# jayleicn/ClipBERT

Hardware: NVIDIA H100
Metric: clips/sec fwd+bwd MSRVTT ret (ResNet50+BERT-base) (higher is better)
Workload: dtype bf16

## Files before the change

### clipbert_b200/csrc/gemm.cu

```cuda
#include <algorithm>

#include "common.cuh"
#include "host_util.h"

namespace cb {

constexpr int BM = 128;
constexpr int BK = 64;
constexpr int CONSUMER_WARPS = 8;
constexpr int GEMM_THREADS = (CONSUMER_WARPS + 1) * 32;
constexpr int PP_THREADS = 3 * 128;
constexpr int PP_PRODUCER_REGS = 40;
constexpr int PP_CONSUMER_REGS = 232;
constexpr int PP_BAR_TURN = 1;
constexpr int MAX_STAGES = 8;
constexpr int SMEM_LIMIT = 232448;
constexpr int STG_PITCH = 36;
constexpr int STG_WARP_FLOATS = 16 * STG_PITCH;
constexpr int EPI_BYTES = CONSUMER_WARPS * STG_WARP_FLOATS * 4;
constexpr int IN_BOX_BYTES = BM * 64 * 2;

struct GemmEpi {
  const float* scale;
  const float* shift;
// ... 215 lines not shown
  const int kc = (K + BK - 1) / BK;
  if (MODE == 1) {
    t.tap = r % ntaps;
    const int split = r / ntaps;
    t.it_begin = split * iters_per_split;
    t.n_iters = min(kc, t.it_begin + iters_per_split) - t.it_begin;
  } else {
    t.tap = 0;
    t.it_begin = 0;
    t.n_iters = ntaps * kc;
  }
  return t;
}

template <int BN, int TA, int TB>
__device__ __forceinline__ void mma_tile(float (&acc)[BN / 2], uint32_t smem0, int stage_bytes, int KCH, int STAGES, int n_iters, int wg,
                                         int lane, int& s, uint32_t& ph, uint64_t* full_bar, uint64_t* empty_bar) {
  using Cfg = GemmCfg<BN>;
  int prev = -1;
  for (int i = 0; i < n_iters; i += KCH) {
    const int nch = min(KCH, n_iters - i);
    mbar_wait(&full_bar[s], ph);
    __syncwarp();
    wgmma_fence();
    wgmma_fence_acc(acc);
    for (int ch = 0; ch < nch; ++ch) {
      const uint32_t a_addr = smem0 + s * stage_bytes + ch * Cfg::STAGE_BYTES + wg * (64 * 128);
      const uint32_t b_addr = smem0 + s * stage_bytes + ch * Cfg::STAGE_BYTES + Cfg::A_BYTES;
#pragma unroll
      for (int k = 0; k < BK / 16; ++k) {
        const uint64_t ad = TA ? gmma_desc(a_addr + k * 2048, BK * 128, 1024) : gmma_desc(a_addr + k * 32, 16, 1024);
        const uint64_t bd = TB ? gmma_desc(b_addr + k * 2048, BK * 128, 1024) : gmma_desc(b_addr + k * 32, 16, 1024);
        wgmma_bf16<BN, TA, TB>(acc, ad, bd, (i > 0 || ch > 0 || k > 0) ? 1u : 0u);
      }
    }
    wgmma_commit();
    wgmma_wait<1>();
    wgmma_fence_acc(acc);
    if (prev >= 0) {
      __syncwarp();
      if (lane == 0) mbar_arrive(&empty_bar[prev]);
    }
    prev = s;
    if (++s == STAGES) { s = 0; ph ^= 1; }
  }
  wgmma_wait<0>();
  wgmma_fence_acc(acc);
  if (prev >= 0) {
    __syncwarp();
    if (lane == 0) mbar_arrive(&empty_bar[prev]);
  }
}

template <int BN, int TB>
__device__ __forceinline__ void mma_tile_pp(float (&acc)[2][BN / 2], uint32_t smem0, int stage_bytes, int KCH, int STAGES, int n_iters,
                                            int lane, int& s, uint32_t& ph, uint64_t* full_bar, uint64_t* empty_bar, int pass_bar,
                                            bool in_stage) {
  using Cfg = GemmCfg<BN>;
  int prev = -1;
  for (int i = 0; i < n_iters; i += KCH) {
    const int nch = min(KCH, n_iters - i);
    mbar_wait_unguarded(&full_bar[s], ph);
    __syncwarp();
    wgmma_fence();
    wgmma_fence_acc(acc[0]);
    wgmma_fence_acc(acc[1]);
    for (int ch = 0; ch < nch; ++ch) {
      const uint32_t a_addr = smem0 + s * stage_bytes + ch * Cfg::STAGE_BYTES;
      const uint32_t b_addr = a_addr + Cfg::A_BYTES;
#pragma unroll
      for (int k = 0; k < BK / 16; ++k) {
        const uint64_t bd = TB ? gmma_desc(b_addr + k * 2048, BK * 128, 1024) : gmma_desc(b_addr + k * 32, 16, 1024);
        const uint32_t accum = (i > 0 || ch > 0 || k > 0) ? 1u : 0u;
#pragma unroll
        for (int h = 0; h < 2; ++h) wgmma_bf16<BN, 0, TB>(acc[h], gmma_desc(a_addr + h * (64 * 128) + k * 32, 16, 1024), bd, accum);
      }
    }
    wgmma_commit();
    wgmma_wait<1>();
    wgmma_fence_acc(acc[0]);
    wgmma_fence_acc(acc[1]);
    if (prev >= 0) {
      __syncwarp();
      mbar_arrive_if(&empty_bar[prev], lane == 0);
    }
    prev = s;
    if (++s == STAGES) { s = 0; ph ^= 1; }
    if (pass_bar && i + KCH >= n_iters) {
      if (in_stage) mbar_wait_unguarded(&full_bar[s], ph);
      named_bar_arrive(pass_bar, 2 * 128);
    }
  }
  wgmma_wait<0>();
  wgmma_fence_acc(acc[0]);
  wgmma_fence_acc(acc[1]);
  if (prev >= 0) {
    __syncwarp();
    mbar_arrive_if(&empty_bar[prev], lane == 0);
  }
}

template <int BN, bool STORE = false>
__device__ __forceinline__ void wgrad_epilogue(const float (&acc)[BN / 2], float* obase, int64_t out_ld, const float* scale, int M, int N, int r0,
                                               int n0, int lane) {
  const int r1 = r0 + 8;
  const float rs0 = (r0 < M && scale) ? scale[r0] : 1.0f;
  const float rs1 = (r1 < M && scale) ? scale[r1] : 1.0f;
#pragma unroll
  for (int j = 0; j < BN / 8; ++j) {
    const int n = n0 + j * 8 + 2 * (lane & 3);
    if (n < N) {
      if constexpr (STORE) {
        if (r0 < M) *reinterpret_cast<float2*>(obase + static_cast<int64_t>(r0) * out_ld + n) = make_float2(acc[4 * j] * rs0, acc[4 * j + 1] * rs0);
        if (r1 < M) *reinterpret_cast<float2*>(obase + static_cast<int64_t>(r1) * out_ld + n) = make_float2(acc[4 * j + 2] * rs1, acc[4 * j + 3] * rs1);
      } else {
        if (r0 < M) red_add_f32x2(obase + static_cast<int64_t>(r0) * out_ld + n, acc[4 * j] * rs0, acc[4 * j + 1] * rs0);
        if (r1 < M) red_add_f32x2(obase + static_cast<int64_t>(r1) * out_ld + n, acc[4 * j + 2] * rs1, acc[4 * j + 3] * rs1);
      }
    }
  }
}

__device__ __forceinline__ uint32_t swz128(uint32_t box, int r, int q) { return box + r * 128 + ((q ^ (r & 7)) << 4); }

template <int BN, int MODE>
__global__ void __launch_bounds__(PP_THREADS, 1)
    gemm_pingpong_kernel(const __grid_constant__ CUtensorMap tmA, const __grid_constant__ CUtensorMap tmB, const __grid_constant__ CUtensorMap tmR,
                         const __grid_constant__ CUtensorMap tmX, int M, int N, int K, int ntaps, int tap_w, int tap_sign, int tiles_m,
                         int tiles_n, int total_tiles, int STAGES, int KCH, int N_IN, GemmEpi epi) {
  static_assert(MODE != 1 && BN <= 128, "TN / NN tiles of 128 x 64 or 128 x 128");
  using Cfg = GemmCfg<BN>;
  extern __shared__ uint8_t smem_raw[];
  uint8_t* smem = reinterpret_cast<uint8_t*>((reinterpret_cast<uintptr_t>(smem_raw) + 1023) & ~static_cast<uintptr_t>(1023));
  const int stage_bytes = KCH * Cfg::STAGE_BYTES;
  const bool has_res = epi.residual != nullptr, has_aux = epi.aux != nullptr;
  constexpr int IN_TILE_BYTES = (BN / 64) * IN_BOX_BYTES;
  const int in_bytes = (has_res + has_aux) * IN_TILE_BYTES;
  uint8_t* in_base = smem + STAGES * stage_bytes;
  uint8_t* stg_base = in_base + N_IN * in_bytes;
  uint64_t* full_bar = reinterpret_cast<uint64_t*>(stg_base + EPI_BYTES);
  uint64_t* empty_bar = full_bar + MAX_STAGES;
  uint64_t* in_full = empty_bar + MAX_STAGES;
  uint64_t* in_empty = in_full + 2;

  const int warp = __shfl_sync(0xffffffffu, static_cast<int>(threadIdx.x >> 5), 0);
  const int lane = threadIdx.x & 31;
  const int unit = blockIdx.x;
  const int n_units = gridDim.x;
  if (threadIdx.x == 0) dbg_stamp(epi, 0);
  pdl_trigger();
  if (threadIdx.x == 0) {
    tma_prefetch_desc(&tmA);
    tma_prefetch_desc(&tmB);
    if (has_res) tma_prefetch_desc(&tmR);
    if (has_aux) tma_prefetch_desc(&tmX);
    for (int s = 0; s < STAGES; ++s) {
      mbar_init(&full_bar[s], 1);
      mbar_init(&empty_bar[s], 4);
    }
    for (int b = 0; b < 2; ++b) {
      mbar_init(&in_full[b], 1);
      mbar_init(&in_empty[b], 4);
    }
    fence_mbar_init();
  }
  __syncthreads();
  const int kc_per_tap = (K + BK - 1) / BK;
  const int n_iters = ntaps * kc_per_tap;
  const bool in_stage = in_bytes && !N_IN;
  const int tile_stages = (n_iters + KCH - 1) / KCH + (in_stage ? 1 : 0);
  pdl_wait();
  if (threadIdx.x == 0) dbg_stamp(epi, 1);

  if (warp < 4) {
    setmaxnreg_dec<PP_PRODUCER_REGS>();
    if (warp == 0 && lane == 0) {
      constexpr int B_BOXES = (MODE == 0) ? 1 : BN / 64;
      int s = 0;
      uint32_t ph = 0;
      auto load_inputs = [&](int tile) {
        const TileInfo t = decode_tile<BN, MODE>(tile, tiles_m, tiles_n, K, ntaps, 0);
        uint64_t* bar;
        uint8_t* dst;
        if (N_IN) {
          const int local = (tile - unit) / n_units;
          const int b = N_IN == 2 ? (local & 1) : 0;
          const int uses = N_IN == 2 ? (local >> 1) : local;
          mbar_wait(&in_empty[b], (static_cast<uint32_t>(uses) & 1u) ^ 1u);
          bar = &in_full[local & 1];
          dst = in_base + b * in_bytes;
        } else {
          mbar_wait(&empty_bar[s], ph ^ 1);
          bar = &full_bar[s];
          dst = smem + s * stage_bytes;
          if (++s == STAGES) { s = 0; ph ^= 1; }
        }
        mbar_expect_tx(bar, in_bytes);
        if (has_res) {
#pragma unroll
          for (int j = 0; j < BN / 64; ++j) tma_load_2d(dst + j * IN_BOX_BYTES, &tmR, bar, t.n0 + j * 64, t.m0);
          dst += IN_TILE_BYTES;
        }
        if (has_aux) {
#pragma unroll
          for (int j = 0; j < BN / 64; ++j) tma_load_2d(dst + j * IN_BOX_BYTES, &tmX, bar, t.n0 + j * 64, t.m0);
        }
      };
      int pend = -1;
      for (int tile = unit; tile < total_tiles; tile += n_units) {
        const TileInfo t = decode_tile<BN, MODE>(tile, tiles_m, tiles_n, K, ntaps, 0);
        const bool inputs_first = tile < unit + N_IN * n_units;
        if (in_bytes && N_IN && inputs_first) load_inputs(tile);
        for (int i = 0; i < n_iters; i += KCH) {
          const int nch = min(KCH, n_iters - i);
          mbar_wait(&empty_bar[s], ph ^ 1);
          mbar_expect_tx(&full_bar[s], nch * Cfg::STAGE_BYTES);
          int tp = 0, kc = i;
          if (ntaps > 1) { tp = i / kc_per_tap; kc = i - tp * kc_per_tap; }
          for (int ch = 0; ch < nch; ++ch) {
            uint8_t* sa = smem + s * stage_bytes + ch * Cfg::STAGE_BYTES;
            uint8_t* sb = sa + Cfg::A_BYTES;
            int shift = 0;
            if (ntaps == 9) shift = tap_sign * ((tp / 3 - 1) * tap_w + (tp % 3 - 1));
            else if (ntaps > 1) shift = tap_sign * tp * tap_w;
            tma_load_2d(sa, &tmA, &full_bar[s], kc * BK, t.m0 + shift);
            if (MODE == 0) {
              tma_load_2d(sb, &tmB, &full_bar[s], tp * K + kc * BK, t.nb0);
            } else if (epi.mn3d) {
              tma_load_3d(sb, &tmB, &full_bar[s], 0, kc * BK, (tp * N + t.nb0) >> 6);
            } else {
#pragma unroll
              for (int j = 0; j < B_BOXES; ++j) tma_load_2d(sb + j * (BK * 128), &tmB, &full_bar[s], tp * N + t.nb0 + j * 64, kc * BK);
            }
            if (++kc == kc_per_tap) { kc = 0; ++tp; }
          }
          if (++s == STAGES) { s = 0; ph ^= 1; }
          if (i == 0 && tile == unit) dbg_stamp(epi, 2);
        }
        if (in_stage) load_inputs(tile);
        if (pend >= 0) load_inputs(pend);
        pend = (in_bytes && N_IN && !inputs_first) ? tile : -1;
      }
      if (pend >= 0) load_inputs(pend);
      dbg_stamp(epi, 3);
    }
    return;
  }

  setmaxnreg_inc<PP_CONSUMER_REGS>();
  const int wg = (warp >> 2) - 1;
  const int wq = warp & 3;
  const uint32_t smem0 = smem_u32(smem);
  const uint64_t dseed = epi.drop_thresh ? drop_seed(epi.seed, epi.seed_off) : 0ull;
  float acc[2][BN / 2];
  int s = 0;
  uint32_t ph = 0;
  auto ring_skip = [&](int n) {
    s += n;
    while (s >= STAGES) { s -= STAGES; ph ^= 1; }
  };
  if (wg == 1) ring_skip(tile_stages);

  const int er = lane & 15, eh = lane >> 4;
  float* stg = reinterpret_cast<float*>(stg_base) + (warp - 4) * STG_WARP_FLOATS;
  const bool has_out2 = epi.out2 != nullptr;
  const bool has_shift = epi.shift != nullptr;
  const bool full = (N & 15) == 0 && epi.scale == nullptr;
  const bool drop = epi.drop_thresh != 0;
  int kind = EK_GENERIC;
  if (full) {
    if (!drop && !has_out2 && !has_aux && (epi.act == CB_ACT_NONE || epi.act == CB_ACT_RELU)) kind = EK_SHIFT_ACT;
    else if (!drop && !has_out2 && !has_shift && has_aux && epi.aux_mode == CB_AUX_RELU_MASK && epi.act == CB_ACT_NONE) kind = EK_RELU_MASK;
    else if (drop && !has_out2 && !has_aux && epi.act == CB_ACT_NONE) kind = EK_DROP_RES;
    else if (!drop && has_out2 && !has_aux && !has_res && epi.act == CB_ACT_GELU_STASH_GRAD) kind = EK_GELU_STASH;
    else if (!drop && !has_out2 && !has_shift && has_aux && epi.aux_mode == CB_AUX_MUL && epi.act == CB_ACT_NONE) kind = EK_AUX_MUL;
  }
  const bool kind_relu = epi.act == CB_ACT_RELU;
  const bool guard = (N & 15) != 0;

  for (int local = wg, tile = unit + wg * n_units; tile < total_tiles; local += 2, tile += 2 * n_units) {
    const TileInfo t = decode_tile<BN, MODE>(tile, tiles_m, tiles_n, K, ntaps, 0);
    if (local > 0) named_bar_sync(PP_BAR_TURN + wg, 2 * 128);
    const int pass = tile + n_units < total_tiles ? PP_BAR_TURN + (wg ^ 1) : 0;
    mma_tile_pp<BN, MODE != 0>(acc, smem0, stage_bytes, KCH, STAGES, n_iters, lane, s, ph, full_bar, empty_bar, pass, in_stage);

    const uint32_t in_buf = N_IN ? smem_u32(in_base) + (N_IN == 2 ? wg : 0) * in_bytes : smem0 + s * stage_bytes;
    if (in_bytes) {
      if (N_IN) mbar_wait_unguarded(&in_full[wg], static_cast<uint32_t>(local >> 1) & 1u);
      else mbar_wait_unguarded(&full_bar[s], ph);
    }
    int orow_half[2];
#pragma unroll
    for (int h = 0; h < 2; ++h) {
      const int m = t.m0 + h * 64 + wq * 16 + er;
      bool row_ok = m < M;
      int64_t orow = m;
      if (epi.rowmap == CB_ROWMAP_PAD) {
        const int hw = epi.H * epi.W;
        const int img = m / hw;
        const int r = m - img * hw;
        const int y = r / epi.W, x = r - y * epi.W;
        orow = (static_cast<int64_t>(img) * (epi.H + 2) + y + 1) * (epi.W + 2) + x + 1;
      } else if (epi.rowmap == CB_ROWMAP_UNPAD) {
        const int wp = epi.W + 2, hp = epi.H + 2;
        const int img = m / (hp * wp);
        const int r = m - img * (hp * wp);
        const int y = r / wp, x = r - y * wp;
        row_ok = row_ok && y >= 1 && y <= epi.H && x >= 1 && x <= epi.W;
        orow = (static_cast<int64_t>(img) * epi.H + (y - 1)) * epi.W + (x - 1);
      }
      orow_half[h] = row_ok ? static_cast<int>(orow) : -1;
    }
#pragma unroll
    for (int sc = 0; sc < BN / 32; ++sc) {
#pragma unroll 1
      for (int h = 0; h < 2; ++h) {
        const int wrow = h * 64 + wq * 16;
        __syncwarp();
#pragma unroll
        for (int jj = 0; jj < 4; ++jj) {
          const int j = sc * 4 + jj;
          float* p = stg + (lane >> 2) * STG_PITCH + jj * 8 + 2 * (lane & 3);
          const bool h1 = h != 0;
          *reinterpret_cast<float2*>(p) = make_float2(h1 ? acc[1][4 * j] : acc[0][4 * j], h1 ? acc[1][4 * j + 1] : acc[0][4 * j + 1]);
          *reinterpret_cast<float2*>(p + 8 * STG_PITCH) =
              make_float2(h1 ? acc[1][4 * j + 2] : acc[0][4 * j + 2], h1 ? acc[1][4 * j + 3] : acc[0][4 * j + 3]);
        }
        __syncwarp();
        const int nb = t.n0 + sc * 32 + eh * 16;
        const int64_t orow = h ? orow_half[1] : orow_half[0];
        if (orow < 0 || nb >= N) continue;
        constexpr int NC = 16;
        float f[NC];
        const uint32_t srow = smem_u32(stg + er * STG_PITCH + eh * 16);
#pragma unroll
        for (int j = 0; j < NC / 4; ++j) {
          const uint4 u = lds128(srow + j * 16);
          f[4 * j] = __uint_as_float(u.x); f[4 * j + 1] = __uint_as_float(u.y);
          f[4 * j + 2] = __uint_as_float(u.z); f[4 * j + 3] = __uint_as_float(u.w);
        }
        uint32_t res16[NC / 2], aux16[NC / 2];
        const int tc = sc * 32 + eh * 16;
        const int q = (tc & 63) >> 3;
        if (has_res) {
#pragma unroll
          for (int j = 0; j < 2; ++j) {
            const uint4 u = lds128(swz128(in_buf + (tc >> 6) * IN_BOX_BYTES, wrow + er, q + j));
            res16[4 * j] = u.x; res16[4 * j + 1] = u.y; res16[4 * j + 2] = u.z; res16[4 * j + 3] = u.w;
          }
        }
        if (has_aux) {
#pragma unroll
          for (int j = 0; j < 2; ++j) {
            const uint4 u = lds128(swz128(in_buf + (has_res ? IN_TILE_BYTES : 0) + (tc >> 6) * IN_BOX_BYTES, wrow + er, q + j));
            aux16[4 * j] = u.x; aux16[4 * j + 1] = u.y; aux16[4 * j + 2] = u.z; aux16[4 * j + 3] = u.w;
          }
        }
        float shv[NC];
        if (has_shift) {
#pragma unroll
          for (int j = 0; j < NC; j += 4) {
            float4 s4 = make_float4(0.f, 0.f, 0.f, 0.f);
            if (nb + j + 4 <= N) s4 = __ldg(reinterpret_cast<const float4*>(epi.shift + nb + j));
            shv[j] = s4.x; shv[j + 1] = s4.y; shv[j + 2] = s4.z; shv[j + 3] = s4.w;
          }
        }
        uint32_t o2_16[NC / 2];
        switch (kind) {
          case EK_SHIFT_ACT: epilogue_shift_act<NC>(f, shv, has_shift, res16, has_res, kind_relu); break;
          case EK_RELU_MASK: epilogue_relu_mask<NC>(f, res16, has_res, aux16); break;
          case EK_DROP_RES:
            epilogue_drop_res<NC>(f, shv, has_shift, res16, has_res, dseed, static_cast<uint64_t>(orow) * static_cast<uint64_t>(N) + nb,
                                  epi.drop_thresh, epi.drop_inv_keep);
            break;
          case EK_GELU_STASH: epilogue_gelu_stash<NC>(f, shv, has_shift, o2_16); break;
          case EK_AUX_MUL: epilogue_aux_mul<NC>(f, res16, has_res, aux16); break;
          default:
            if (guard) epilogue_math<NC, true>(f, epi, shv, has_shift, dseed, nb, N, orow, res16, has_res, aux16, has_aux, o2_16, has_out2);
            else epilogue_math<NC, false>(f, epi, shv, has_shift, dseed, nb, N, orow, res16, has_res, aux16, has_aux, o2_16, has_out2);
        }
        if (epi.out_fp32) {
          float* o = reinterpret_cast<float*>(epi.out) + orow * epi.out_ld + nb;
#pragma unroll
          for (int j = 0; j < NC; j += 4)
            if (nb + j + 4 <= N) *reinterpret_cast<float4*>(o + j) = make_float4(f[j], f[j + 1], f[j + 2], f[j + 3]);
        } else {
          __nv_bfloat16* o = reinterpret_cast<__nv_bfloat16*>(epi.out) + orow * epi.out_ld + nb;
#pragma unroll
          for (int j = 0; j < 2; ++j)
            if (nb + 8 * j + 8 <= N)
              *reinterpret_cast<uint4*>(o + 8 * j) = make_uint4(pack_bf16x2(f[8 * j], f[8 * j + 1]), pack_bf16x2(f[8 * j + 2], f[8 * j + 3]),
                                                                pack_bf16x2(f[8 * j + 4], f[8 * j + 5]), pack_bf16x2(f[8 * j + 6], f[8 * j + 7]));
        }
        if (has_out2) {
          __nv_bfloat16* o = epi.out2 + orow * epi.out2_ld + nb;
#pragma unroll
          for (int j = 0; j < 2; ++j)
            if (nb + 8 * j + 8 <= N) *reinterpret_cast<uint4*>(o + 8 * j) = make_uint4(o2_16[4 * j], o2_16[4 * j + 1], o2_16[4 * j + 2], o2_16[4 * j + 3]);
        }
      }
    }
    if (in_bytes) {
      __syncwarp();
      if (lane == 0) mbar_arrive(N_IN ? &in_empty[N_IN == 2 ? wg : 0] : &empty_bar[s]);
      if (!N_IN && ++s == STAGES) { s = 0; ph ^= 1; }
    }
    ring_skip(tile_stages);
  }
  if (threadIdx.x == 4 * 32) dbg_stamp(epi, 11);
}

template <int BN, bool DET = false>
__global__ void __launch_bounds__(GEMM_THREADS, 1)
    gemm_kernel(const __grid_constant__ CUtensorMap tmA, const __grid_constant__ CUtensorMap tmB, int M, int N, int K, int ntaps, int tap_w,
                int tap_sign, int iters_per_split, int tiles_m, int tiles_n, int total_tiles, int STAGES, int KCH, GemmEpi epi, float* ws) {
  using Cfg = GemmCfg<BN>;
  extern __shared__ uint8_t smem_raw[];
  uint8_t* smem = reinterpret_cast<uint8_t*>((reinterpret_cast<uintptr_t>(smem_raw) + 1023) & ~static_cast<uintptr_t>(1023));
  const int stage_bytes = KCH * Cfg::STAGE_BYTES;
  uint64_t* full_bar = reinterpret_cast<uint64_t*>(smem + STAGES * stage_bytes);
  uint64_t* empty_bar = full_bar + MAX_STAGES;

  const int warp = __shfl_sync(0xffffffffu, static_cast<int>(threadIdx.x >> 5), 0);
  const int lane = threadIdx.x & 31;
  const int unit = blockIdx.x;
  const int n_units = gridDim.x;
  if (threadIdx.x == 0) dbg_stamp(epi, 0);
  pdl_trigger();
  if (threadIdx.x == 0) {
    tma_prefetch_desc(&tmA);
    tma_prefetch_desc(&tmB);
    for (int s = 0; s < STAGES; ++s) {
      mbar_init(&full_bar[s], 1);
      mbar_init(&empty_bar[s], CONSUMER_WARPS);
    }
    fence_mbar_init();
  }
  __syncthreads();
  pdl_wait();
  if (threadIdx.x == 0) dbg_stamp(epi, 1);

  if (warp >= CONSUMER_WARPS) {
    if (warp == CONSUMER_WARPS && lane == 0) {
      int s = 0;
      uint32_t ph = 0;
      for (int tile = unit; tile < total_tiles; tile += n_units) {
        const TileInfo t = decode_tile<BN, 1>(tile, tiles_m, tiles_n, K, ntaps, iters_per_split);
        int shift = 0;
        if (ntaps == 9) shift = tap_sign * ((t.tap / 3 - 1) * tap_w + (t.tap % 3 - 1));
        for (int i = 0; i < t.n_iters; i += KCH) {
          const int nch = min(KCH, t.n_iters - i);
          mbar_wait(&empty_bar[s], ph ^ 1);
          mbar_expect_tx(&full_bar[s], nch * Cfg::STAGE_BYTES);
          int kit = t.it_begin + i;
          for (int ch = 0; ch < nch; ++ch, ++kit) {
            uint8_t* sa = smem + s * stage_bytes + ch * Cfg::STAGE_BYTES;
            uint8_t* sb = sa + Cfg::A_BYTES;
            const int p = kit * BK;
            if (epi.mn3d) {
              tma_load_3d(sa, &tmA, &full_bar[s], 0, p, t.m0 >> 6);
              tma_load_3d(sb, &tmB, &full_bar[s], 0, p + shift, t.nb0 >> 6);
            } else {
// ... 86 lines not shown
  const SmemPlan none = plan_ring(bn, staging, kiters, force_kch, 0, 0);
  if (in_bytes == 0) return none;
  const SmemPlan two = plan_ring(bn, staging, kiters, force_kch, in_bytes, 2);
  if (two.stages >= 2 && two.stages * two.kch >= kiters) return two;
  if (kiters > 4 && none.stages >= 2 && none.kch * none.chunk_bytes >= in_bytes) return none;
  return plan_ring(bn, staging, kiters, force_kch, in_bytes, 1);
}
static int epi_in_bytes(const cb_gemm_desc& d, int bn) {
  return d.mode == CB_GEMM_WGRAD ? 0 : ((d.residual != nullptr) + (d.aux != nullptr)) * (bn / 64) * IN_BOX_BYTES;
}

static int real_splits(int kc, int want) {
  const int sp = want < 1 ? 1 : (want > kc ? kc : want);
  return ceil_div(kc, ceil_div(kc, sp));
}

struct SplitReduceJob {
  float* out;
  const float* ws;
  int64_t out_ld;
  int M, W, S;
};
struct SplitReduce {
  int njobs;
  SplitReduceJob j[8];
};
__global__ void __launch_bounds__(256) wgrad_split_reduce_kernel(const __grid_constant__ SplitReduce r) {
  pdl_wait();
  pdl_trigger();
  const SplitReduceJob& J = r.j[blockIdx.y];
  const int w4 = J.W / 4;
  const int64_t total = static_cast<int64_t>(J.M) * w4, plane = static_cast<int64_t>(J.M) * J.W;
  for (int64_t i = static_cast<int64_t>(blockIdx.x) * 256 + threadIdx.x; i < total; i += static_cast<int64_t>(gridDim.x) * 256) {
    const int64_t m = i / w4;
    const int c = static_cast<int>(i - m * w4) * 4;
    float4* o = reinterpret_cast<float4*>(J.out + m * J.out_ld + c);
    float4 v = *o;
    const float* p = J.ws + m * J.W + c;
    for (int s = 0; s < J.S; ++s) {
      const float4 a = *reinterpret_cast<const float4*>(p + s * plane);
      v.x += a.x; v.y += a.y; v.z += a.z; v.w += a.w;
    }
    *o = v;
  }
}
static int launch_split_reduce(const SplitReduce& r, cudaStream_t stream, const char* what) {
  int64_t most = 0;
  for (int i = 0; i < r.njobs; ++i) most = std::max(most, static_cast<int64_t>(r.j[i].M) * (r.j[i].W / 4));
  const int gx = static_cast<int>(std::min<int64_t>(1024, (most + 255) / 256));
  launch_k(wgrad_split_reduce_kernel, dim3(gx, r.njobs), 256, 0, stream, r);
  return check_launch(what);
}

template <int BN, int MODE, bool DET = false>
static int launch_gemm(const cb_gemm_desc& d, const GemmEpi& epi_in, cudaStream_t stream, float* ws = nullptr) {
  static_assert(MODE == 1 || BN <= 128, "TN / NN: 128 x 64 or 128 x 128 tiles");
  static_assert(MODE == 1 || !DET, "only the weight gradients have a deterministic instantiation");
  GemmEpi epi = epi_in;
  using Cfg = GemmCfg<BN>;
  static bool attr_set = false;
  auto kern = [] {
    if constexpr (MODE == 1) return gemm_kernel<BN, DET>;
    else return gemm_pingpong_kernel<BN, MODE>;
  }();
  if (!attr_set) {
    cudaError_t e = cudaFuncSetAttribute(kern, cudaFuncAttributeMaxDynamicSharedMemorySize, SMEM_LIMIT);
    if (e != cudaSuccess) {
      set_error("cudaFuncSetAttribute(smem=%d): %s", SMEM_LIMIT, cudaGetErrorString(e));
      return CB_ERR_CUDA;
    }
    attr_set = true;
  }
  alignas(64) CUtensorMap ta, tb, tr, tx;
  bool mn3d = false;
  int iters_per_split = 0;
  const int tiles_m = ceil_div(d.m, BM), tiles_n = ceil_div(d.n, BN);
  int total = tiles_m * tiles_n;
  int kiters;
  bool ok;
  if (MODE == 0) {
    ok = get_tmap_2d(&ta, d.a, d.k, d.a_rows, d.a_ld, BK, BM) &&
         get_tmap_2d(&tb, d.b, static_cast<uint64_t>(d.k) * d.ntaps, d.b_rows, d.b_ld, BK, BN);
    kiters = ceil_div(d.k, BK) * d.ntaps;
  } else if (MODE == 2) {
    ok = get_tmap_2d(&ta, d.a, d.k, d.a_rows, d.a_ld, BK, BM);
    mn3d = g_mn3d && d.n % 64 == 0 &&
           get_tmap_3d_mn(&tb, d.b, static_cast<uint64_t>(d.n) * d.ntaps, d.b_rows, d.b_ld, BK, BN / 64);
    if (!mn3d) ok = ok && get_tmap_2d(&tb, d.b, static_cast<uint64_t>(d.n) * d.ntaps, d.b_rows, d.b_ld, 64, BK);
    kiters = ceil_div(d.k, BK) * d.ntaps;
  } else {
    mn3d = g_mn3d && d.m % 64 == 0 && d.n % 64 == 0 && get_tmap_3d_mn(&ta, d.a, d.m, d.a_rows, d.a_ld, BK, BM / 64) &&
           get_tmap_3d_mn(&tb, d.b, d.n, d.b_rows, d.b_ld, BK, BN / 64);
    ok = mn3d || (get_tmap_2d(&ta, d.a, d.m, d.a_rows, d.a_ld, 64, BK) && get_tmap_2d(&tb, d.b, d.n, d.b_rows, d.b_ld, 64, BK));
    const int kc = ceil_div(d.k, BK);
    iters_per_split = ceil_div(kc, real_splits(kc, d.split_k));
    total *= real_splits(kc, d.split_k) * d.ntaps;
    kiters = iters_per_split;
  }
  tr = ta;
  tx = ta;
  if (MODE != 1 && d.residual) ok = ok && get_tmap_2d(&tr, d.residual, d.n, d.m, d.res_ld, 64, BM);
  if (MODE != 1 && d.aux) ok = ok && get_tmap_2d(&tx, d.aux, d.n, d.m, d.aux_ld, 64, BM);
  if (!ok) return CB_ERR_CUDA;
  epi.mn3d = mn3d ? 1 : 0;
  const int units = sm_count();
  const int grid = total < units ? total : units;
  const int in_bytes = epi_in_bytes(d, BN);
  const SmemPlan sp = plan_smem(BN, MODE != 1, kiters, (d.reserved >> 8) & 15, in_bytes);
  const int kch = sp.kch, stages = sp.stages;
  if (stages < 2) {
    set_error("cb_gemm: not enough shared memory for a 2-stage pipeline (BN=%d, epilogue %d B + inputs %d B)", BN, sp.epi_bytes,
              in_bytes);
    return CB_ERR_INVALID;
  }
  const int smem_bytes = stages * kch * Cfg::STAGE_BYTES + sp.n_in * in_bytes + sp.epi_bytes + Cfg::BAR_BYTES + 1024;
  if constexpr (MODE == 1)
    launch_gemm_k(kern, grid, GEMM_THREADS, smem_bytes, stream, ta, tb, d.m, d.n, d.k, d.ntaps, d.tap_w, d.tap_sign, iters_per_split,
                  tiles_m, tiles_n, total, stages, kch, epi, ws);
  else
    launch_gemm_k(kern, grid, PP_THREADS, smem_bytes, stream, ta, tb, tr, tx, d.m, d.n, d.k, d.ntaps, d.tap_w, d.tap_sign, tiles_m,
                  tiles_n, total, stages, kch, sp.n_in, epi);
  return check_launch("cb_gemm");
}

struct LaunchCfg {
  int bn, splits;
};

static LaunchCfg choose_config(const cb_gemm_desc& d, int units) {
  const int kc = ceil_div(d.k, BK);
  const bool wgrad = d.mode == CB_GEMM_WGRAD;
  const int block_n = (!wgrad && d.block_n == 256) ? 128 : d.block_n;
  static const int cand[3] = {64, 128, 256};
  LaunchCfg best = {64, 1};
  double best_cost = 1e30;
  for (int c = 0; c < 3; ++c) {
    const int bn = cand[c];
    if (block_n && bn != block_n) continue;
    if (!wgrad && bn == 256) continue;
    if (bn > 64 && d.n <= bn / 2) continue;
    const int64_t base = static_cast<int64_t>(ceil_div(d.m, BM)) * ceil_div(d.n, bn) * (wgrad ? d.ntaps : 1);
    const int max_split = wgrad ? (d.split_k > 0 ? d.split_k : (kc < 32 ? kc : 32)) : 1;
    for (int sp = (wgrad && d.split_k > 0) ? d.split_k : 1; sp <= max_split; ++sp) {
      const int ips = ceil_div(wgrad ? kc : kc * d.ntaps, sp);
      const int real_sp = wgrad ? ceil_div(kc, ips) : 1;
      const int64_t tiles = base * real_sp;
      const double rounds = static_cast<double>((tiles + units - 1) / units);
      const SmemPlan pl = plan_smem(bn, !wgrad, ips, (d.reserved >> 8) & 15, epi_in_bytes(d, bn));
      if (pl.stages < 2) continue;
      const double shallow = (pl.stages * pl.kch < 3 && ips > 2) ? 3.0 : 1.0;
      const double stage_cost = 450.0 + pl.kch * pl.chunk_bytes / 60.0;
      const double main_loop = ceil_div(ips, pl.kch) * stage_cost * shallow;
      double cost;
      if (wgrad) {
        cost = rounds * (main_loop + bn * 24.0) + 2500.0;
      } else {
        const double epi = bn * 30.0;
        const double per_tile = main_loop > 0.5 * (main_loop + epi) ? main_loop : 0.5 * (main_loop + epi);
        cost = rounds * per_tile + 0.5 * epi + 2500.0;
      }
      if (cost < best_cost) {
        best_cost = cost;
        best = {bn, real_sp};
      }
    }
  }
  return best;
}

constexpr int WG_MAX_PROBLEMS = 8;
struct WgradProblem {
  CUtensorMap tmA, tmB;
  float* out;
  const float* scale;
  int64_t out_ld;
  int M, N, K;
  int ntaps, tap_w, tap_sign;
  int iters_per_split, tiles_m, tiles_n;
  int tile_begin;
  int mn3d;
};
struct WgradGroup {
  int nprob, total_tiles;
  WgradProblem p[WG_MAX_PROBLEMS];
};
struct WgradWorkspace {
  float* p[WG_MAX_PROBLEMS];
};
struct WgTile {
  int pi, m0, n0, tap, it_begin, n_iters;
};
__device__ __forceinline__ WgTile wg_decode(const WgradGroup& g, int tile) {
  WgTile t;
  int pi = 0;
  while (pi + 1 < g.nprob && tile >= g.p[pi + 1].tile_begin) ++pi;
  const WgradProblem& P = g.p[pi];
  int r = tile - P.tile_begin;
  const int nt = r % P.tiles_n;
  r /= P.tiles_n;
  const int mt = r % P.tiles_m;
  r /= P.tiles_m;
  t.pi = pi;
  t.m0 = mt * BM;
  t.tap = r % P.ntaps;
  const int split = r / P.ntaps;
  const int kc = (P.K + BK - 1) / BK;
  t.it_begin = split * P.iters_per_split;
  t.n_iters = min(kc, t.it_begin + P.iters_per_split) - t.it_begin;
  t.n0 = nt;
  return t;
}

template <int BN, bool DET = false>
__global__ void __launch_bounds__(GEMM_THREADS, 1)
    wgrad_group_kernel(const __grid_constant__ WgradGroup g, int STAGES, int KCH, const __grid_constant__ WgradWorkspace ws) {
  using Cfg = GemmCfg<BN>;
  extern __shared__ uint8_t smem_raw[];
  uint8_t* smem = reinterpret_cast<uint8_t*>((reinterpret_cast<uintptr_t>(smem_raw) + 1023) & ~static_cast<uintptr_t>(1023));
// ... 189 lines not shown
extern "C" int cb_gemm(const cb_gemm_desc* dp, void* stream_v) {
  using namespace cb;
  CB_REQUIRE(dp != nullptr, "cb_gemm: null descriptor");
  const cb_gemm_desc& d = *dp;
  cudaStream_t stream = static_cast<cudaStream_t>(stream_v);
  CB_REQUIRE(d.a && d.b && d.out, "cb_gemm: null operand pointer");
  CB_REQUIRE(d.m > 0 && d.n > 0 && d.k > 0, "cb_gemm: empty problem m=%d n=%d k=%d", d.m, d.n, d.k);
  CB_REQUIRE(d.ntaps == 1 || d.ntaps == 9 || (d.ntaps == 4 && d.mode == CB_GEMM_TN),
             "cb_gemm: ntaps must be 1, 9 (3x3 conv) or 4 (row taps, TN only) (got %d)", d.ntaps);
  CB_REQUIRE(d.mode == CB_GEMM_TN || d.mode == CB_GEMM_WGRAD || d.mode == CB_GEMM_NN, "cb_gemm: bad mode %d", d.mode);
  CB_REQUIRE(d.dropout_p >= 0.0f && d.dropout_p <= 1.0f, "cb_gemm: dropout_p %g outside [0, 1]", d.dropout_p);

  GemmEpi epi;
  epi.scale = d.scale;
  epi.shift = d.shift;
  epi.residual = static_cast<const __nv_bfloat16*>(d.residual);
  epi.aux = static_cast<const __nv_bfloat16*>(d.aux);
  epi.aux_mode = d.aux ? d.aux_mode : CB_AUX_NONE;
  epi.act = d.act;
  epi.out = d.out;
  epi.out_ld = d.out_ld;
  epi.out_fp32 = d.out_fp32;
  epi.out2 = static_cast<__nv_bfloat16*>(d.out2);
  epi.out2_ld = d.out2_ld;
  epi.rowmap = d.rowmap;
  epi.H = d.map_h;
  epi.W = d.map_w;
  epi.seed = d.dropout_seed;
  epi.dbg = g_gemm_timeline;
  epi.mn3d = 0;
  {
    const DropCfg dc = make_drop(d.dropout_p, d.dropout_seed);
    epi.drop_thresh = dc.thresh;
    epi.drop_inv_keep = dc.inv_keep;
    epi.seed_off = dc.offset;
  }

  if (d.mode == CB_GEMM_TN || d.mode == CB_GEMM_NN) {
    const bool nn = d.mode == CB_GEMM_NN;
    CB_REQUIRE(d.n % 8 == 0, "cb_gemm(TN): n must be a multiple of 8 (got %d)", d.n);
    CB_REQUIRE(d.k % 8 == 0, "cb_gemm(TN): k must be a multiple of 8 (got %d)", d.k);
    CB_REQUIRE(d.out_ld % 8 == 0, "cb_gemm(TN): out_ld must be a multiple of 8");
    CB_REQUIRE(!d.residual || d.res_ld % 8 == 0, "cb_gemm(TN): res_ld must be a multiple of 8");
    CB_REQUIRE(!d.aux || d.aux_ld % 8 == 0, "cb_gemm(TN): aux_ld must be a multiple of 8");
    CB_REQUIRE((reinterpret_cast<uintptr_t>(d.residual) & 15) == 0, "cb_gemm(TN): residual must be 16-byte aligned");
    CB_REQUIRE((reinterpret_cast<uintptr_t>(d.aux) & 15) == 0, "cb_gemm(TN): aux must be 16-byte aligned");
    CB_REQUIRE(!d.out2 || d.out2_ld % 8 == 0, "cb_gemm(TN): out2_ld must be a multiple of 8");
    CB_REQUIRE(!(d.out2 && d.out_fp32), "cb_gemm(TN): out2 requires a bf16 primary output");
    CB_REQUIRE(d.rowmap == CB_ROWMAP_NONE || (d.map_h > 0 && d.map_w > 0), "cb_gemm: rowmap needs map_h/map_w");
    CB_REQUIRE(d.ntaps == 1 || d.tap_w > 2, "cb_gemm: tap modes need tap_w (padded row pitch in pixels)");
    CB_REQUIRE(d.block_n == 0 || d.block_n == 64 || d.block_n == 128 || d.block_n == 256, "cb_gemm: block_n must be 0, 64, 128 or 256 (got %d)",
               d.block_n);
    const LaunchCfg lc = choose_config(d, sm_count());
    switch (lc.bn) {
      case 64: return nn ? launch_gemm<64, 2>(d, epi, stream) : launch_gemm<64, 0>(d, epi, stream);
      case 128: return nn ? launch_gemm<128, 2>(d, epi, stream) : launch_gemm<128, 0>(d, epi, stream);
      default: CB_REQUIRE(false, "cb_gemm: no tile width for block_n %d", d.block_n);
    }
  } else {
    CB_REQUIRE(d.out_fp32 == 1, "cb_gemm(WGRAD): output must be fp32");
    CB_REQUIRE(d.m % 8 == 0 && d.n % 8 == 0, "cb_gemm(WGRAD): m, n must be multiples of 8 (got %d, %d)", d.m, d.n);
    CB_REQUIRE(d.out_ld % 4 == 0, "cb_gemm(WGRAD): out_ld must be a multiple of 4");
    CB_REQUIRE((reinterpret_cast<uintptr_t>(d.out) & 15) == 0, "cb_gemm(WGRAD): out must be 16-byte aligned");
    const LaunchCfg lc = choose_config(d, plan_sm_count());
    cb_gemm_desc d2 = d;
    d2.split_k = lc.splits;
    if (g_det.load(std::memory_order_relaxed) && lc.splits > 1) {
      const int64_t need = wgrad_ws_bytes(d, lc.splits);
      CB_REQUIRE(d.workspace != nullptr && d.workspace_bytes >= need && (reinterpret_cast<uintptr_t>(d.workspace) & 15) == 0,
                 "cb_gemm(WGRAD): deterministic mode needs a 16-byte aligned workspace of %lld bytes (cb_gemm_workspace_bytes), got %lld",
                 static_cast<long long>(need), static_cast<long long>(d.workspace ? d.workspace_bytes : 0));
      float* ws = static_cast<float*>(d.workspace);
      int rc = CB_ERR_INVALID;
      switch (lc.bn) {
        case 64: rc = launch_gemm<64, 1, true>(d2, epi, stream, ws); break;
        case 128: rc = launch_gemm<128, 1, true>(d2, epi, stream, ws); break;
        case 256: rc = launch_gemm<256, 1, true>(d2, epi, stream, ws); break;
        default: CB_REQUIRE(false, "cb_gemm(WGRAD): block_n must be 0, 64, 128 or 256 (got %d)", lc.bn);
      }
      if (rc != CB_OK) return rc;
      SplitReduce red;
      red.njobs = 1;
      red.j[0] = {static_cast<float*>(d.out), ws, d.out_ld, d.m, d.ntaps * d.n, lc.splits};
      return launch_split_reduce(red, stream, "cb_gemm(split reduce)");
    }
    switch (lc.bn) {
      case 64: return launch_gemm<64, 1>(d2, epi, stream);
      case 128: return launch_gemm<128, 1>(d2, epi, stream);
      case 256: return launch_gemm<256, 1>(d2, epi, stream);
      default: CB_REQUIRE(false, "cb_gemm(WGRAD): block_n must be 0, 64, 128 or 256 (got %d)", lc.bn);
    }
  }
  return CB_ERR_INVALID;
}

extern "C" int cb_gemm_wgrad_group(const cb_gemm_desc* descs, int n, void* stream_v) {
  using namespace cb;
  CB_REQUIRE(descs != nullptr && n >= 1, "cb_gemm_wgrad_group: no problems");
  cudaStream_t stream = static_cast<cudaStream_t>(stream_v);
  for (int i = 0; i < n; ++i) {
    const cb_gemm_desc& d = descs[i];
    CB_REQUIRE(d.mode == CB_GEMM_WGRAD && d.out_fp32 == 1, "cb_gemm_wgrad_group: problem %d is not an fp32 WGRAD descriptor", i);
    CB_REQUIRE(d.a && d.b && d.out && d.m > 0 && d.n > 0 && d.k > 0, "cb_gemm_wgrad_group: problem %d: null operand / empty shape", i);
    CB_REQUIRE(d.m % 8 == 0 && d.n % 8 == 0 && d.out_ld % 4 == 0 && (reinterpret_cast<uintptr_t>(d.out) & 15) == 0,
               "cb_gemm_wgrad_group: problem %d: m, n multiples of 8, out 16-byte aligned, out_ld a multiple of 4", i);
    CB_REQUIRE(d.ntaps == 1 || d.ntaps == 9, "cb_gemm_wgrad_group: problem %d: ntaps must be 1 or 9", i);
  }
  const bool det = g_det.load(std::memory_order_relaxed);
  int64_t need = 0;
  if (det) {
    need = group_ws_bytes(descs, n);
// ... 43 lines not shown
```

### clipbert_b200/ops.py

```python
import ctypes

import torch

from . import _lib as L
from ._lib import (ACT_GELU, ACT_GELU_STASH_GRAD, ACT_NONE, ACT_RELU, ACT_TANH, AUX_GELU_GRAD, AUX_MUL, AUX_NONE,
                   AUX_RELU_MASK, AUX_TANH_GRAD, CB_GEMM_TN, CB_GEMM_WGRAD, ROWMAP_NONE, ROWMAP_PAD, ROWMAP_UNPAD)

CB_GEMM_NN = 2
_c = ctypes
_vp, _i, _i64, _f, _u64 = _c.c_void_p, _c.c_int, _c.c_int64, _c.c_float, _c.c_uint64

_SIGS = {
    "cb_layernorm_fwd": [_vp, _vp, _vp, _vp, _vp, _i, _i, _f, _vp],
    "cb_layernorm_bwd": [_vp, _vp, _vp, _vp, _vp, _vp, _vp, _vp, _vp, _i, _i, _f, _u64, _vp],
    "cb_embed_text_fwd": [_vp, _vp, _vp, _vp, _vp, _vp, _vp, _vp, _i, _i, _i, _i, _i, _f, _f, _u64, _vp],
    "cb_embed_text_bwd": [_vp] * 12 + [_i, _i, _i, _i, _i, _f, _u64, _vp],
    "cb_embed_visual_fwd": [_vp, _vp, _i, _vp, _vp, _vp, _vp, _vp, _vp, _vp, _i, _i, _i, _i, _i, _i, _i, _f, _f, _u64, _vp],
    "cb_embed_visual_bwd": [_vp, _vp, _vp, _vp, _i] + [_vp] * 12 + [_i, _i, _i, _i, _i, _i, _i, _i, _f, _u64, _vp],
    "cb_colsum": [_vp, _i64, _vp, _i, _i, _vp],
    "cb_dropout": [_vp, _vp, _i64, _f, _u64, _vp],
    "cb_dropout_offset_advance": [_vp, _vp, _vp],
    "cb_gelu_bwd": [_vp, _vp, _vp, _i64, _vp],
    "cb_pad_cast": [_vp, _i64, _vp, _i, _i, _i, _vp],
    "cb_cast_scale": [_vp, _vp, _i64, _vp, _i64, _vp],
# ... 226 lines not shown
            if k in _GEMM_PTR_FIELDS:
                v = _p(v) if isinstance(v, torch.Tensor) else v
            setattr(d, k, v)
    return arr


def gemm_workspace_bytes(kw):
    return int(L.lib().cb_gemm_workspace_bytes(_gemm_descs([kw])))


def gemm_wgrad_group_workspace_bytes(kws):
    return int(L.lib().cb_gemm_wgrad_group_workspace_bytes(_gemm_descs(kws), len(kws)))


def _with_workspace(kw, nbytes):
    if nbytes <= 0:
        return kw
    ws, nb = _scratch_args(nbytes, kw["out"])
    return dict(kw, workspace=ws, workspace_bytes=nb)


def _launch_gemm(name, kws):
    arr = _gemm_descs(kws)
    timing = _gemm_timing is not None or _op_timing is not None
    if timing:
        e0, e1 = torch.cuda.Event(enable_timing=True), torch.cuda.Event(enable_timing=True)
        e0.record()
    if name == "cb_gemm":
        rc = L.lib().cb_gemm(arr, _s())
    else:
        rc = L.lib().cb_gemm_wgrad_group(arr, len(kws), _s())
    if rc != 0:
        raise RuntimeError("%s failed (%d): %s" % (name, rc, L.lib().cb_last_error().decode()))
    if timing:
        e1.record()
        if _gemm_timing is not None:
            _gemm_timing.append((e0, e1))
        if _op_timing is not None:
            d = arr[0]
            label = ("gemm mode=%d m=%d n=%d k=%d taps=%d res=%d aux=%d o2=%d f32=%d rm=%d" % (
                d.mode, d.m, d.n, d.k, d.ntaps, bool(d.residual), bool(d.aux), bool(d.out2), d.out_fp32, d.rowmap)
                if name == "cb_gemm" else "gemm wgrad group x%d" % len(kws))
            _op_timing.append((label, e0, e1))


def gemm(**kw):
    if _tuning is None:
        _load_tuning()
    if _gemm_record is not None:
        _gemm_record.append(dict(kw))
    if _tuning and "block_n" not in kw and "reserved" not in kw:
        t = _tuning.get(gemm_key(kw))
        if t is not None:
            kw = dict(kw, block_n=t[0], split_k=t[1], reserved=(t[2] << 8) | (32 if (len(t) > 3 and t[3]) else 0))
    if kw.get("mode", CB_GEMM_TN) == CB_GEMM_WGRAD and deterministic():
        kw = _with_workspace(kw, gemm_workspace_bytes(kw))
    _launch_gemm("cb_gemm", [kw])


group_wgrad = 3


def gemm_wgrad_group(kws):
    if not kws:
        return
    if len(kws) == 1:
        for kw in kws:
            gemm(**kw)
        return
    if _gemm_record is not None:
        _gemm_record.append(dict(group=[dict(kw) for kw in kws]))
    kws = list(kws)
    if deterministic():
        kws[0] = _with_workspace(kws[0], gemm_wgrad_group_workspace_bytes(kws))
    _launch_gemm("cb_gemm_wgrad_group", kws)


def wgrad_split(m, n, k, ntaps=1, block_n=128):
    return 0


def layernorm_fwd(x, gamma, beta, y, stats, eps):
    _call("cb_layernorm_fwd", _p(x), _p(gamma), _p(beta), _p(y), _p(stats), x.shape[0], x.shape[1], eps, _s())


def layernorm_bwd(dy, x, stats, gamma, dx, dx_drop, dgamma, dbeta, dbias_drop, p, seed):
    if (dgamma is not None or dbeta is not None or dbias_drop is not None) and deterministic():
        layernorm_bwd_det(dy, x, stats, gamma, dx, dx_drop, dgamma, dbeta, dbias_drop, p, seed,
                          _scratch(layernorm_bwd_scratch_bytes(x.shape[0]), x))
        return
    _call("cb_layernorm_bwd", _p(dy), _p(x), _p(stats), _p(gamma), _p(dx), _p(dx_drop), _p(dgamma), _p(dbeta),
          _p(dbias_drop), x.shape[0], x.shape[1], p, seed, _s())


def layernorm_bwd_scratch_bytes(m):
    return int(_fn("cb_layernorm_bwd_scratch_bytes")(m))


def layernorm_bwd_det(dy, x, stats, gamma, dx, dx_drop, dgamma, dbeta, dbias_drop, p, seed, scratch):
    _call("cb_layernorm_bwd_det", _p(dy), _p(x), _p(stats), _p(gamma), _p(dx), _p(dx_drop), _p(dgamma), _p(dbeta),
          _p(dbias_drop), x.shape[0], x.shape[1], p, seed, _p(scratch), scratch.numel() * 4, _s())


def embed_text_fwd(ids, word, pos, type0, gamma, beta, out, stats, nseq, lt, l, eps, p, seed):
    _call("cb_embed_text_fwd", _p(ids), _p(word), _p(pos), _p(type0), _p(gamma), _p(beta), _p(out), _p(stats), nseq, lt, l,
          word.shape[0], word.shape[1], eps, p, seed, _s())

# ... 194 lines not shown
```

Baseline: 3987.

## Add cooperative two-warpgroup GEMM kernel for TN/NN with 128x256 tiles

```diff
diff --git a/clipbert_b200/csrc/gemm.cu b/clipbert_b200/csrc/gemm.cu
--- a/clipbert_b200/csrc/gemm.cu
+++ b/clipbert_b200/csrc/gemm.cu
@@ -291,10 +291,10 @@
   }
 }
 
-template <int BN, int TB>
-__device__ __forceinline__ void mma_tile_pp(float (&acc)[2][BN / 2], uint32_t smem0, int stage_bytes, int KCH, int STAGES, int n_iters,
-                                            int lane, int& s, uint32_t& ph, uint64_t* full_bar, uint64_t* empty_bar, int pass_bar,
-                                            bool in_stage) {
+template <int BN, int TB, int NH>
+__device__ __forceinline__ void mma_tile_pp(float (&acc)[NH][BN / 2], uint32_t a_off, uint32_t smem0, int stage_bytes, int KCH, int STAGES,
+                                            int n_iters, int lane, int& s, uint32_t& ph, uint64_t* full_bar, uint64_t* empty_bar,
+                                            int pass_bar, bool in_stage) {
   using Cfg = GemmCfg<BN>;
   int prev = -1;
   for (int i = 0; i < n_iters; i += KCH) {
@@ -302,23 +302,23 @@
     mbar_wait_unguarded(&full_bar[s], ph);
     __syncwarp();
     wgmma_fence();
-    wgmma_fence_acc(acc[0]);
-    wgmma_fence_acc(acc[1]);
+#pragma unroll
+    for (int h = 0; h < NH; ++h) wgmma_fence_acc(acc[h]);
     for (int ch = 0; ch < nch; ++ch) {
-      const uint32_t a_addr = smem0 + s * stage_bytes + ch * Cfg::STAGE_BYTES;
-      const uint32_t b_addr = a_addr + Cfg::A_BYTES;
+      const uint32_t a_addr = smem0 + s * stage_bytes + ch * Cfg::STAGE_BYTES + a_off;
+      const uint32_t b_addr = smem0 + s * stage_bytes + ch * Cfg::STAGE_BYTES + Cfg::A_BYTES;
 #pragma unroll
       for (int k = 0; k < BK / 16; ++k) {
         const uint64_t bd = TB ? gmma_desc(b_addr + k * 2048, BK * 128, 1024) : gmma_desc(b_addr + k * 32, 16, 1024);
         const uint32_t accum = (i > 0 || ch > 0 || k > 0) ? 1u : 0u;
 #pragma unroll
-        for (int h = 0; h < 2; ++h) wgmma_bf16<BN, 0, TB>(acc[h], gmma_desc(a_addr + h * (64 * 128) + k * 32, 16, 1024), bd, accum);
+        for (int h = 0; h < NH; ++h) wgmma_bf16<BN, 0, TB>(acc[h], gmma_desc(a_addr + h * (64 * 128) + k * 32, 16, 1024), bd, accum);
       }
     }
     wgmma_commit();
     wgmma_wait<1>();
-    wgmma_fence_acc(acc[0]);
-    wgmma_fence_acc(acc[1]);
+#pragma unroll
+    for (int h = 0; h < NH; ++h) wgmma_fence_acc(acc[h]);
     if (prev >= 0) {
       __syncwarp();
       mbar_arrive_if(&empty_bar[prev], lane == 0);
@@ -331,8 +331,8 @@
     }
   }
   wgmma_wait<0>();
-  wgmma_fence_acc(acc[0]);
-  wgmma_fence_acc(acc[1]);
+#pragma unroll
+  for (int h = 0; h < NH; ++h) wgmma_fence_acc(acc[h]);
   if (prev >= 0) {
     __syncwarp();
     mbar_arrive_if(&empty_bar[prev], lane == 0);
@@ -362,12 +362,13 @@
 
 __device__ __forceinline__ uint32_t swz128(uint32_t box, int r, int q) { return box + r * 128 + ((q ^ (r & 7)) << 4); }
 
-template <int BN, int MODE>
-__global__ void __launch_bounds__(PP_THREADS, 1)
-    gemm_pingpong_kernel(const __grid_constant__ CUtensorMap tmA, const __grid_constant__ CUtensorMap tmB, const __grid_constant__ CUtensorMap tmR,
-                         const __grid_constant__ CUtensorMap tmX, int M, int N, int K, int ntaps, int tap_w, int tap_sign, int tiles_m,
-                         int tiles_n, int total_tiles, int STAGES, int KCH, int N_IN, GemmEpi epi) {
-  static_assert(MODE != 1 && BN <= 128, "TN / NN tiles of 128 x 64 or 128 x 128");
+template <int BN, int MODE, bool COOP>
+__device__ __forceinline__ void gemm_tn_nn_body(const CUtensorMap& tmA, const CUtensorMap& tmB, const CUtensorMap& tmR, const CUtensorMap& tmX,
+                                                int M, int N, int K, int ntaps, int tap_w, int tap_sign, int tiles_m, int tiles_n,
+                                                int total_tiles, int STAGES, int KCH, int N_IN, const GemmEpi& epi) {
+  static_assert(MODE != 1 && (COOP ? (BN == 128 || BN == 256) : BN <= 128), "TN / NN: ping-pong 128 x 64 / 128, cooperative 128 x 128 / 256");
+  constexpr int READERS = COOP ? 8 : 4;
+  constexpr int NH = COOP ? 1 : 2;
   using Cfg = GemmCfg<BN>;
   extern __shared__ uint8_t smem_raw[];
   uint8_t* smem = reinterpret_cast<uint8_t*>((reinterpret_cast<uintptr_t>(smem_raw) + 1023) & ~static_cast<uintptr_t>(1023));
@@ -395,11 +396,11 @@
     if (has_aux) tma_prefetch_desc(&tmX);
     for (int s = 0; s < STAGES; ++s) {
       mbar_init(&full_bar[s], 1);
-      mbar_init(&empty_bar[s], 4);
+      mbar_init(&empty_bar[s], READERS);
     }
     for (int b = 0; b < 2; ++b) {
       mbar_init(&in_full[b], 1);
-      mbar_init(&in_empty[b], 4);
+      mbar_init(&in_empty[b], READERS);
     }
     fence_mbar_init();
   }
@@ -491,14 +492,14 @@
   const int wq = warp & 3;
   const uint32_t smem0 = smem_u32(smem);
   const uint64_t dseed = epi.drop_thresh ? drop_seed(epi.seed, epi.seed_off) : 0ull;
-  float acc[2][BN / 2];
+  float acc[NH][BN / 2];
   int s = 0;
   uint32_t ph = 0;
   auto ring_skip = [&](int n) {
     s += n;
     while (s >= STAGES) { s -= STAGES; ph ^= 1; }
   };
-  if (wg == 1) ring_skip(tile_stages);
+  if (!COOP && wg == 1) ring_skip(tile_stages);
 
   const int er = lane & 15, eh = lane >> 4;
   float* stg = reinterpret_cast<float*>(stg_base) + (warp - 4) * STG_WARP_FLOATS;
@@ -517,15 +518,18 @@
   const bool kind_relu = epi.act == CB_ACT_RELU;
   const bool guard = (N & 15) != 0;
 
-  for (int local = wg, tile = unit + wg * n_units; tile < total_tiles; local += 2, tile += 2 * n_units) {
+  constexpr int TILE_STEP = COOP ? 1 : 2;
+  for (int local = COOP ? 0 : wg, tile = unit + local * n_units; tile < total_tiles; local += TILE_STEP, tile += TILE_STEP * n_units) {
     const TileInfo t = decode_tile<BN, MODE>(tile, tiles_m, tiles_n, K, ntaps, 0);
-    if (local > 0) named_bar_sync(PP_BAR_TURN + wg, 2 * 128);
-    const int pass = tile + n_units < total_tiles ? PP_BAR_TURN + (wg ^ 1) : 0;
-    mma_tile_pp<BN, MODE != 0>(acc, smem0, stage_bytes, KCH, STAGES, n_iters, lane, s, ph, full_bar, empty_bar, pass, in_stage);
-
-    const uint32_t in_buf = N_IN ? smem_u32(in_base) + (N_IN == 2 ? wg : 0) * in_bytes : smem0 + s * stage_bytes;
+    if (!COOP && local > 0) named_bar_sync(PP_BAR_TURN + wg, 2 * 128);
+    const int pass = (!COOP && tile + n_units < total_tiles) ? PP_BAR_TURN + (wg ^ 1) : 0;
+    mma_tile_pp<BN, MODE != 0, NH>(acc, COOP ? wg * (64 * 128) : 0, smem0, stage_bytes, KCH, STAGES, n_iters, lane, s, ph, full_bar,
+                                   empty_bar, pass, in_stage);
+
+    const int ib = COOP ? (local & 1) : wg;
+    const uint32_t in_buf = N_IN ? smem_u32(in_base) + (N_IN == 2 ? ib : 0) * in_bytes : smem0 + s * stage_bytes;
     if (in_bytes) {
-      if (N_IN) mbar_wait_unguarded(&in_full[wg], static_cast<uint32_t>(local >> 1) & 1u);
+      if (N_IN) mbar_wait_unguarded(&in_full[ib], static_cast<uint32_t>(local >> 1) & 1u);
       else mbar_wait_unguarded(&full_bar[s], ph);
     }
     int orow_half[2];
@@ -553,17 +557,18 @@
 #pragma unroll
     for (int sc = 0; sc < BN / 32; ++sc) {
 #pragma unroll 1
-      for (int h = 0; h < 2; ++h) {
+      for (int h = COOP ? wg : 0; h < (COOP ? wg + 1 : 2); ++h) {
         const int wrow = h * 64 + wq * 16;
         __syncwarp();
 #pragma unroll
         for (int jj = 0; jj < 4; ++jj) {
           const int j = sc * 4 + jj;
           float* p = stg + (lane >> 2) * STG_PITCH + jj * 8 + 2 * (lane & 3);
-          const bool h1 = h != 0;
-          *reinterpret_cast<float2*>(p) = make_float2(h1 ? acc[1][4 * j] : acc[0][4 * j], h1 ? acc[1][4 * j + 1] : acc[0][4 * j + 1]);
+          const bool h1 = !COOP && h != 0;
+          *reinterpret_cast<float2*>(p) =
+              make_float2(h1 ? acc[NH - 1][4 * j] : acc[0][4 * j], h1 ? acc[NH - 1][4 * j + 1] : acc[0][4 * j + 1]);
           *reinterpret_cast<float2*>(p + 8 * STG_PITCH) =
-              make_float2(h1 ? acc[1][4 * j + 2] : acc[0][4 * j + 2], h1 ? acc[1][4 * j + 3] : acc[0][4 * j + 3]);
+              make_float2(h1 ? acc[NH - 1][4 * j + 2] : acc[0][4 * j + 2], h1 ? acc[NH - 1][4 * j + 3] : acc[0][4 * j + 3]);
         }
         __syncwarp();
         const int nb = t.n0 + sc * 32 + eh * 16;
@@ -641,12 +646,27 @@
     }
     if (in_bytes) {
       __syncwarp();
-      if (lane == 0) mbar_arrive(N_IN ? &in_empty[N_IN == 2 ? wg : 0] : &empty_bar[s]);
+      if (lane == 0) mbar_arrive(N_IN ? &in_empty[N_IN == 2 ? ib : 0] : &empty_bar[s]);
       if (!N_IN && ++s == STAGES) { s = 0; ph ^= 1; }
     }
-    ring_skip(tile_stages);
+    if (!COOP) ring_skip(tile_stages);
   }
   if (threadIdx.x == 4 * 32) dbg_stamp(epi, 11);
+}
+
+template <int BN, int MODE>
+__global__ void __launch_bounds__(PP_THREADS, 1)
+    gemm_pingpong_kernel(const __grid_constant__ CUtensorMap tmA, const __grid_constant__ CUtensorMap tmB, const __grid_constant__ CUtensorMap tmR,
+                         const __grid_constant__ CUtensorMap tmX, int M, int N, int K, int ntaps, int tap_w, int tap_sign, int tiles_m,
+                         int tiles_n, int total_tiles, int STAGES, int KCH, int N_IN, GemmEpi epi) {
+  gemm_tn_nn_body<BN, MODE, false>(tmA, tmB, tmR, tmX, M, N, K, ntaps, tap_w, tap_sign, tiles_m, tiles_n, total_tiles, STAGES, KCH, N_IN, epi);
+}
+template <int BN, int MODE>
+__global__ void __launch_bounds__(PP_THREADS, 1)
+    gemm_coop_kernel(const __grid_constant__ CUtensorMap tmA, const __grid_constant__ CUtensorMap tmB, const __grid_constant__ CUtensorMap tmR,
+                     const __grid_constant__ CUtensorMap tmX, int M, int N, int K, int ntaps, int tap_w, int tap_sign, int tiles_m,
+                     int tiles_n, int total_tiles, int STAGES, int KCH, int N_IN, GemmEpi epi) {
+  gemm_tn_nn_body<BN, MODE, true>(tmA, tmB, tmR, tmX, M, N, K, ntaps, tap_w, tap_sign, tiles_m, tiles_n, total_tiles, STAGES, KCH, N_IN, epi);
 }
 
 template <int BN, bool DET = false>
@@ -839,15 +859,17 @@
   return check_launch(what);
 }
 
-template <int BN, int MODE, bool DET = false>
+template <int BN, int MODE, bool DET = false, bool COOP = false>
 static int launch_gemm(const cb_gemm_desc& d, const GemmEpi& epi_in, cudaStream_t stream, float* ws = nullptr) {
-  static_assert(MODE == 1 || BN <= 128, "TN / NN: 128 x 64 or 128 x 128 tiles");
+  static_assert(MODE == 1 || (COOP ? BN >= 128 : BN <= 128), "TN / NN: ping-pong 128 x 64 / 128, cooperative 128 x 128 / 256");
   static_assert(MODE == 1 || !DET, "only the weight gradients have a deterministic instantiation");
+  static_assert(MODE != 1 || !COOP, "the weight-gradient kernel is always cooperative");
   GemmEpi epi = epi_in;
   using Cfg = GemmCfg<BN>;
   static bool attr_set = false;
   auto kern = [] {
     if constexpr (MODE == 1) return gemm_kernel<BN, DET>;
+    else if constexpr (COOP) return gemm_coop_kernel<BN, MODE>;
     else return gemm_pingpong_kernel<BN, MODE>;
   }();
   if (!attr_set) {
@@ -912,19 +934,25 @@
 
 struct LaunchCfg {
   int bn, splits;
+  bool coop;
 };
+
+constexpr int RESERVED_COOP = 1 << 12;
 
 static LaunchCfg choose_config(const cb_gemm_desc& d, int units) {
   const int kc = ceil_div(d.k, BK);
   const bool wgrad = d.mode == CB_GEMM_WGRAD;
-  const int block_n = (!wgrad && d.block_n == 256) ? 128 : d.block_n;
-  static const int cand[3] = {64, 128, 256};
-  LaunchCfg best = {64, 1};
+  const bool force_coop = (d.reserved & RESERVED_COOP) != 0;
+  static const int cand_bn[4] = {64, 128, 128, 256};
+  static const bool cand_coop[4] = {false, false, true, true};
+  LaunchCfg best = {0, 1, false};
   double best_cost = 1e30;
-  for (int c = 0; c < 3; ++c) {
-    const int bn = cand[c];
-    if (block_n && bn != block_n) continue;
-    if (!wgrad && bn == 256) continue;
+  for (int c = 0; c < 4; ++c) {
+    const int bn = cand_bn[c];
+    const bool coop = !wgrad && cand_coop[c];
+    if (wgrad && c == 2) continue;
+    if (d.block_n && bn != d.block_n) continue;
+    if (!wgrad && coop != (force_coop || bn == 256) && (force_coop || d.block_n)) continue;
     if (bn > 64 && d.n <= bn / 2) continue;
     const int64_t base = static_cast<int64_t>(ceil_div(d.m, BM)) * ceil_div(d.n, bn) * (wgrad ? d.ntaps : 1);
     const int max_split = wgrad ? (d.split_k > 0 ? d.split_k : (kc < 32 ? kc : 32)) : 1;
@@ -935,12 +963,16 @@
       const double rounds = static_cast<double>((tiles + units - 1) / units);
       const SmemPlan pl = plan_smem(bn, !wgrad, ips, (d.reserved >> 8) & 15, epi_in_bytes(d, bn));
       if (pl.stages < 2) continue;
+      if (coop && pl.stages < 3 && pl.stages * pl.kch < ips) continue;
       const double shallow = (pl.stages * pl.kch < 3 && ips > 2) ? 3.0 : 1.0;
       const double stage_cost = 450.0 + pl.kch * pl.chunk_bytes / 60.0;
       const double main_loop = ceil_div(ips, pl.kch) * stage_cost * shallow;
       double cost;
       if (wgrad) {
         cost = rounds * (main_loop + bn * 24.0) + 2500.0;
+      } else if (coop) {
+        const double epi = bn * 30.0 * (d.out2 ? 3.0 : 1.0);
+        cost = rounds * (0.75 * main_loop + epi) + 2500.0 + 40000.0;
       } else {
         const double epi = bn * 30.0;
         const double per_tile = main_loop > 0.5 * (main_loop + epi) ? main_loop : 0.5 * (main_loop + epi);
@@ -948,9 +980,15 @@
       }
       if (cost < best_cost) {
         best_cost = cost;
-        best = {bn, real_sp};
+        best = {bn, real_sp, coop};
       }
     }
+  }
+  if (best.bn == 0 && (d.block_n || force_coop)) {
+    cb_gemm_desc any = d;
+    any.block_n = 0;
+    any.reserved &= ~RESERVED_COOP;
+    return choose_config(any, units);
   }
   return best;
 }
@@ -1246,11 +1284,20 @@
     CB_REQUIRE(d.block_n == 0 || d.block_n == 64 || d.block_n == 128 || d.block_n == 256, "cb_gemm: block_n must be 0, 64, 128 or 256 (got %d)",
                d.block_n);
     const LaunchCfg lc = choose_config(d, sm_count());
-    switch (lc.bn) {
-      case 64: return nn ? launch_gemm<64, 2>(d, epi, stream) : launch_gemm<64, 0>(d, epi, stream);
-      case 128: return nn ? launch_gemm<128, 2>(d, epi, stream) : launch_gemm<128, 0>(d, epi, stream);
-      default: CB_REQUIRE(false, "cb_gemm: no tile width for block_n %d", d.block_n);
-    }
+    if (lc.coop) {
+      switch (lc.bn) {
+        case 128: return nn ? launch_gemm<128, 2, false, true>(d, epi, stream) : launch_gemm<128, 0, false, true>(d, epi, stream);
+        case 256: return nn ? launch_gemm<256, 2, false, true>(d, epi, stream) : launch_gemm<256, 0, false, true>(d, epi, stream);
+        default: break;
+      }
+    } else {
+      switch (lc.bn) {
+        case 64: return nn ? launch_gemm<64, 2>(d, epi, stream) : launch_gemm<64, 0>(d, epi, stream);
+        case 128: return nn ? launch_gemm<128, 2>(d, epi, stream) : launch_gemm<128, 0>(d, epi, stream);
+        default: break;
+      }
+    }
+    CB_REQUIRE(false, "cb_gemm: no launch plan for block_n %d (reserved 0x%x)", d.block_n, d.reserved);
   } else {
     CB_REQUIRE(d.out_fp32 == 1, "cb_gemm(WGRAD): output must be fp32");
     CB_REQUIRE(d.m % 8 == 0 && d.n % 8 == 0, "cb_gemm(WGRAD): m, n must be multiples of 8 (got %d, %d)", d.m, d.n);
diff --git a/clipbert_b200/ops.py b/clipbert_b200/ops.py
--- a/clipbert_b200/ops.py
+++ b/clipbert_b200/ops.py
@@ -302,7 +302,7 @@
     if _tuning and "block_n" not in kw and "reserved" not in kw:
         t = _tuning.get(gemm_key(kw))
         if t is not None:
-            kw = dict(kw, block_n=t[0], split_k=t[1], reserved=(t[2] << 8) | (32 if (len(t) > 3 and t[3]) else 0))
+            kw = dict(kw, block_n=t[0], split_k=t[1], reserved=(t[2] << 8) | ((1 << 12) if (len(t) > 3 and t[3]) else 0))
     if kw.get("mode", CB_GEMM_TN) == CB_GEMM_WGRAD and deterministic():
         kw = _with_workspace(kw, gemm_workspace_bytes(kw))
     _launch_gemm("cb_gemm", [kw])
```

Result: faster. 4031 (median of 6 runs) (+1.1%).
